# heyblackC/DFMIR

Hardware: AMD Instinct MI355X
Metric: train-step image-pairs/sec (fwd+bwd): 2D 256x256 bs=16 and 3D 160^3 bs=1 (higher is better)
Workload: dtype f32 (fp16x2-split MFMA, fp32 accumulate)

## Files before the change

dfmir_amd/_lib.py:

```python
import ctypes
import os
from ctypes import c_float, c_int, c_longlong, c_void_p, POINTER, Structure

_HERE = os.path.dirname(os.path.abspath(__file__))
LIB_PATH = os.environ.get("DFMIR_HIP_LIB") or os.path.join(_HERE, "libdfmir_hip.so")


class DfConvGeom(Structure):
    _fields_ = [(n, c_int) for n in (
        "N", "Cin", "Cout", "Di", "Hi", "Wi", "Do", "Ho", "Wo", "KD", "KH", "KW",
        "stride", "dil", "pd", "ph", "pw", "pad_mode", "act")] + [("slope", c_float)]


P = c_void_p
_GP = POINTER(DfConvGeom)
_SIGS = {
    "dfmir_abi_version": [],
    "dfmir_set_option": [ctypes.c_char_p, ctypes.c_char_p],
    "dfmir_get_option": [ctypes.c_char_p, ctypes.c_char_p, c_int],
    "dfmir_conv_fwd": [_GP, P, P, P, P, P],
    "dfmir_conv_wgrad": [_GP, P, P, P, P],
    "dfmir_bias_grad": [P, P, c_int, c_int, c_longlong, P],
    "dfmir_weight_pack": [P, P, c_int, c_int, c_int, c_int, P],
    "dfmir_weight_pack_floats": [c_int, c_int, c_int],
    "dfmir_weight_pack_batch": [P, c_int, P, c_int, P],
    "dfmir_conv3x3_res_ok": [_GP],
    "dfmir_conv3x3_fwd_scaled_res": [_GP, P, P, c_int, P, P, P, P, c_int, P, P],
    "dfmir_conv3x3_reflect_ring_ok": [_GP],
    "dfmir_conv3x3_reflect_ring_len": [_GP],
    "dfmir_conv3x3_reflect_ring": [_GP, P, P, P, c_int, P, P, P],
    "dfmir_conv_fwd_scaled": [_GP, P, P, c_int, P, P, P, P],
    "dfmir_conv_wgrad_scaled": [_GP, P, P, c_int, P, P, c_int, P, P, P],
    "dfmir_conv_wgrad_scaled_ch": [_GP, P, P, c_int, P, P, c_int, P, P, P, P],
    "dfmir_instnorm_bwd_pmax_ok": [c_longlong],
    "dfmir_instnorm_bwd_pmax": [P, P, P, P, P, c_int, c_longlong, c_int, P, P, c_int, P, P],
    "dfmir_patch_gather_bwd_gp": [P, P, P, c_int, c_int, c_longlong, c_int, c_int, P, P, P],
    "dfmir_patch_gather_bwd_any": [P, P, P, c_int, c_int, c_longlong, c_int, c_int, P, P, P],
    "dfmir_absmax": [P, c_longlong, P, P],
    "dfmir_conv3d_split_ok": [_GP],
    "dfmir_conv3d_split_ws_floats": [c_int, c_int],
    "dfmir_conv3d_split_fwd": [_GP, P, P, c_int, P, P, P, P, P, P],
    "dfmir_conv3d_split_fwd_sub": [_GP, P, P, c_int, P, P, P, P, P, c_int, P],
    "dfmir_conv3d_split_fwd_actgrad": [_GP, P, P, c_int, P, P, P, P, P, c_int, P, c_float, P],
    "dfmir_conv3d_up_ok": [c_int] * 6,
    "dfmir_conv3d_wsplit_batch": [P, c_int, P],
    "dfmir_conv3d_split_is_pair": [c_int],
    "dfmir_conv3d_march_ok": [_GP],
    "dfmir_conv3d_march_fwd": [_GP, P, P, c_int, P, P, P, P, P, c_float, P],
    "dfmir_conv3d_tiny_ok": [_GP],
    "dfmir_conv3d_tiny_fwd": [_GP, P, P, P, P, P, P, c_float, P],
    "dfmir_conv3d_s2c2_ok": [_GP],
    "dfmir_conv3d_s2c2_fwd": [_GP, P, P, P, P, P, P],
    "dfmir_conv3d_s2c2_wgrad": [_GP, P, P, P, P],
    "dfmir_conv3d_s2_ok": [_GP],
    "dfmir_conv3d_s2_fwd": [_GP, P, P, P, P, P, P],
    "dfmir_conv3d_s2_wgrad": [_GP, P, P, P, P, P],
    "dfmir_conv3d_s2_dgrad_ok": [_GP],
    "dfmir_conv3d_s2_dgrad": [_GP, P, P, P, P],
    "dfmir_conv3d_up_ws_floats": [c_int, c_int],
    "dfmir_conv3d_up_fwd": [P, P, c_int, P, c_int, P, P] + [c_int] * 6 + [P],
    "dfmir_conv3d_up_skip2_fwd": [P, P, c_int, P, P, c_int, c_int, P, P, P, P, P] + [c_int] * 7 + [c_float, P],
    "dfmir_conv3d_up_dgrad_ws_floats": [c_int, c_int],
    "dfmir_conv3d_up_dgrad": [P, P, c_int, P, c_int, P, P, P, P, c_float] + [c_int] * 6 + [P],
    "dfmir_conv3d_split_fwd_add": [_GP, P, P, c_int, P, c_int, c_int, P, P, P, P, P],
    "dfmir_conv3d_split_wgrad_ok": [_GP],
    "dfmir_conv3d_split_wgrad": [_GP, P, P, c_int, P, P, c_int, P, P],
    "dfmir_conv3d_split_wgrad_upcat": [_GP, P, P, c_int, P, c_int, P, P, c_int, P, P, P],
    "dfmir_conv3d_upwgrad_ok": [_GP, c_int],
    "dfmir_conv3d_wgrad_is_march": [_GP],
    "dfmir_conv3d_wgrad_is_march_at": [_GP, P, P],
    "dfmir_conv3d_upwgrad_ws_floats": [],
    "dfmir_conv3d_upwgrad": [_GP, P, P, c_int, P, c_int, P, P, c_int, P, P, P, P],
    "dfmir_conv3d_split_wgrad_db": [_GP, P, P, c_int, P, P, c_int, P, P, P],
    "dfmir_probe_merge": [P, P, P, P],
    "dfmir_act_bwd_amax": [P, P, P, c_longlong, c_int, c_float, P, P],
    "dfmir_weight_unpack": [P, P, c_int, c_int, c_int, P],
    "dfmir_weight_unpack_add_batch": [P, c_int, c_longlong, P],
    "dfmir_conv7x7_c1_fwd": [P, P, P, P, c_int, c_int, c_int, c_int, c_int, P],
    "dfmir_conv7x7_c1_wgrad": [P, P, P, P, c_int, c_int, c_int, c_int, c_int, P],
    "dfmir_tapstack_fwd": [P, P] + [c_int] * 7 + [P],
    "dfmir_tapstack_bwd": [P, P] + [c_int] * 7 + [P],
    "dfmir_tapsum_fwd": [P, P, P] + [c_int] * 10 + [c_float, P],
    "dfmir_tapsum_bwd": [P, P] + [c_int] * 9 + [P],
    "dfmir_instnorm_fwd": [P, P, P, P, P, c_int, c_longlong, c_float, c_int, P, P],
    "dfmir_instnorm_stats_ok": [c_longlong],
    "dfmir_instnorm_stats": [P, P, P, c_int, c_longlong, c_float, c_int, P, P],
    "dfmir_instnorm_bwd": [P, P, P, P, P, c_int, c_longlong, c_int, P, P],
    "dfmir_instnorm_bwd_cols_ok": [c_longlong, c_int],
    "dfmir_instnorm_bwd_cols": [P, P, P, P, P, c_int, c_longlong, c_int, P, P, c_int, P],
    "dfmir_in_relu_blurdown_ok": [c_int, c_int],
    "dfmir_in_relu_blurdown_fwd": [P, P, P, P, c_int, c_int, c_int, c_float, P, P],
    "dfmir_in_relu_blurdown_bwd": [P, P, P, P, P, c_int, c_int, c_int, P, P, P],
    "dfmir_act_bwd": [P, P, P, c_longlong, c_int, c_float, P],
    "dfmir_blur_down_fwd": [P, P, c_int, c_int, c_int, P],
    "dfmir_blur_down_bwd": [P, P, c_int, c_int, c_int, P],
    "dfmir_blur_up_fwd": [P, P, c_int, c_int, c_int, P],
    "dfmir_blur_up_bwd": [P, P, c_int, c_int, c_int, P],
    "dfmir_reflect_pad2d_fwd": [P, P, c_int, c_int, c_int, c_int, P],
    "dfmir_reflect_pad2d_bwd": [P, P, c_int, c_int, c_int, c_int, P],
    "dfmir_reflect_pad2d_bwd_add": [P, P, P, c_int, c_int, c_int, c_int, P],
    "dfmir_upcat_fwd": [P, P, P] + [c_int] * 7 + [P],
    "dfmir_upcat_bwd": [P, P, P] + [c_int] * 7 + [P],
    "dfmir_cat_channels_fwd": [P, P, P, c_longlong, c_longlong, c_longlong, P],
    "dfmir_cat_channels_bwd": [P, P, P, c_longlong, c_longlong, c_longlong, P],
    "dfmir_scale": [P, P, c_longlong, c_float, P],
    "dfmir_warp2d_fwd": [P, P, P] + [c_int] * 6 + [P],
    "dfmir_warp2d_bwd": [P, P, P, P, P] + [c_int] * 6 + [P],
    "dfmir_warp3d_fwd": [P, P, P] + [c_int] * 7 + [P],
    "dfmir_warp3d_bwd": [P, P, P, P, P] + [c_int] * 7 + [P],
    "dfmir_warp_bwd_own_ws_floats": [c_int] * 6,
    "dfmir_warp_bwd_own": [c_int, P, P, P, P, P] + [c_int] * 7 + [P, P],
    "dfmir_resize_fwd": [P, P] + [c_int] * 7 + [c_float, P],
    "dfmir_resize_bwd": [P, P] + [c_int] * 7 + [c_float, P],
    "dfmir_resize_bwd_ws_floats": [c_int] * 7,
    "dfmir_resize_bwd_sep": [P, P] + [c_int] * 7 + [c_float, P, P],
    "dfmir_patch_gather_fwd": [P, P, P, c_int, c_int, c_longlong, c_int, P],
    "dfmir_patch_gather_bwd": [P, P, P, c_int, c_int, c_longlong, c_int, P],
    "dfmir_patch_gather_bwd_amax": [P, P, P, c_int, c_int, c_longlong, c_int, P, P],
    "dfmir_patch_gather_fwd_g": [P, P, P, c_int, c_int, c_longlong, c_int, c_int, P],
    "dfmir_patch_gather_bwd_g": [P, P, P, c_int, c_int, c_longlong, c_int, c_int, P, P],
    "dfmir_l2norm_fwd": [P, P, P, c_int, c_longlong, c_float, P],
    "dfmir_l2norm_bwd": [P, P, P, P, c_int, c_longlong, c_float, P],
    "dfmir_patchnce_fwd": [P, P, P, P, c_longlong, c_int, c_int, c_float, P],
    "dfmir_patchnce_bwd": [P, P, P, P, c_longlong, c_int, c_int, c_float, P],
    "dfmir_masked_l1_fwd": [P, P, P, c_float, P, P, c_longlong, P],
    "dfmir_masked_l1_bwd": [P, P, P, c_float, P, P, P, P, c_longlong, P],
    "dfmir_flow_smooth_ws_floats": [],
    "dfmir_flow_smooth_fwd": [P, P, P] + [c_int] * 5 + [P],
    "dfmir_flow_smooth_bwd": [P, P, P] + [c_int] * 5 + [P],
    "dfmir_flow_smooth_fwd_p": [P, P, P] + [c_int] * 6 + [P],
    "dfmir_flow_smooth_bwd_p": [P, P, P] + [c_int] * 6 + [P],
    "dfmir_mul": [P, P, P, c_longlong, P],
    "dfmir_nmi_ws_floats": [c_longlong, c_int],
    "dfmir_nmi_fwd": [P, P, P, P, c_int, c_float, c_float, c_longlong, P, P, P],
    "dfmir_nmi_bwd": [P, P, P, P, c_int, c_float, c_float, c_longlong, P, P, P, P, P],
    "dfmir_ncc_fwd_m": [P, P, P, c_int, P, P, P, P] + [c_int] * 5 + [c_float, P],
    "dfmir_ncc_bwd_m": [P, P, P, c_int, P, P, P, P, P, P] + [c_int] * 5 + [c_float, P],
    "dfmir_ncc_fwd": [P, P, P, P, P, P] + [c_int] * 5 + [c_float, P],
    "dfmir_ncc_bwd": [P, P, P, P, P, P, P, P] + [c_int] * 5 + [c_float, P],
    "dfmir_patch_gather_fwd_multi": [P, c_int, P, P, c_int, c_int, c_longlong, c_int, P],
    "dfmir_nce_head_fwd": [P, c_int, P, P, P, P, P, P, P, P, P, P, c_int, c_int, c_longlong, c_int, c_float, P],
    "dfmir_patch_ids_draw": [P, P, c_int, c_int, c_int, P, P],
    "dfmir_segment_means_fwd": [P, P, c_int, c_int, c_longlong, c_float, P],
    "dfmir_segment_means_bwd": [P, P, c_int, c_int, c_longlong, c_float, P],
    "dfmir_scalar_combine_fwd": [P, c_int, P, c_int, P, P],
    "dfmir_scalar_combine_bwd": [P, c_int, P, c_int, P, P],
    "dfmir_det_head_floats": [],
    "dfmir_det_begin": [P, c_longlong, P, c_longlong, P, c_int, P, c_longlong, P, c_int, ctypes.c_double, P],
    "dfmir_det_end": [P, P, c_longlong, P, c_longlong, P],
    "dfmir_fill_zero": [P, c_longlong, P],
    "dfmir_sum_scaled": [P, P, c_longlong, c_float, P],
    "dfmir_fill_from_scalar": [P, P, c_longlong, c_float, P],
    "dfmir_adam_step": [P, P, P, P, c_longlong] + [c_float] * 7 + [P],
}

_lib = None


class DfmirHipError(RuntimeError):
    pass


def lib():
    global _lib
    if _lib is None:
        import torch
        if not os.path.exists(LIB_PATH):
            raise DfmirHipError(
                "libdfmir_hip.so not found at %s -- build it with `python -c 'import __graft_entry__ as g; "
                "g.build()'` or `make -C dfmir_amd/csrc` (there is no CPU fallback)" % LIB_PATH)
        h = ctypes.CDLL(LIB_PATH)
        for name, args in _SIGS.items():
            fn = getattr(h, name)
            fn.argtypes = args
            fn.restype = c_int
        h.dfmir_weight_pack_floats.restype = c_longlong
        h.dfmir_conv3d_split_ws_floats.restype = c_longlong
        h.dfmir_conv3d_up_ws_floats.restype = c_longlong
        h.dfmir_conv3d_up_dgrad_ws_floats.restype = c_longlong
        h.dfmir_conv3d_upwgrad_ws_floats.restype = c_longlong
        h.dfmir_flow_smooth_ws_floats.restype = c_longlong
        h.dfmir_nmi_ws_floats.restype = c_longlong
        h.dfmir_warp_bwd_own_ws_floats.restype = c_longlong
        h.dfmir_resize_bwd_ws_floats.restype = c_longlong
        h.dfmir_last_error.argtypes = []
        h.dfmir_last_error.restype = ctypes.c_char_p
        _lib = h
    return _lib


def check(rc):
    if rc != 0:
        msg = lib().dfmir_last_error()
        raise DfmirHipError(msg.decode() if msg else "dfmir_hip error %d" % rc)


def set_option(name, value=None):
    check(lib().dfmir_set_option(name.encode(), None if value is None else str(value).encode()))


def get_option(name):
    buf = ctypes.create_string_buffer(256)
    n = lib().dfmir_get_option(name.encode(), buf, 256)
    return None if n < 0 else buf.value.decode()


def exported_symbols():
    return sorted(list(_SIGS.keys()) + ["dfmir_last_error"])
```

dfmir_amd/csrc/taps.hip:

```cpp
#include "common.h"

__device__ __forceinline__ int pre_images(int i, int n, int pad, int pad_mode, int* rp) {
  int cnt = 0;
  rp[cnt++] = i;
  if (pad_mode == 1) {
    if (i >= 1 && i <= pad) rp[cnt++] = -i;
    if (i <= n - 2 && i >= n - 1 - pad) rp[cnt++] = 2 * (n - 1) - i;
  }
  return cnt;
}
__device__ __forceinline__ bool map_coord(int c, int n, int pad_mode, int& out) {
  if (pad_mode == 1) {
    if (c < 0) c = -c;
    if (c >= n) c = 2 * (n - 1) - c;
    out = c < 0 ? 0 : (c >= n ? n - 1 : c);
    return true;
  }
  out = c;
  return (unsigned)c < (unsigned)n;
}

__global__ void tapstack_fwd_k(const float* __restrict__ x, float* __restrict__ s, int N, int C, int H, int W,
                               int K, int pad, int pad_mode) {
  const int T = K * K;
// ... 173 lines not shown
  const int co = mb * 32 + l31;
  float a[25];
#pragma unroll
  for (int s2 = 0; s2 < 25; ++s2) {
    const int t = 2 * s2 + lhi;
    a[s2] = (t < S7_T && co < Cout) ? w[co * S7_T + t] : 0.f;
  }
  __syncthreads();
  st_f32x16 acc[S7_RW];
#pragma unroll
  for (int j = 0; j < S7_RW; ++j)
#pragma unroll
    for (int r = 0; r < 16; ++r) acc[j][r] = 0.f;
#pragma unroll
  for (int s2 = 0; s2 < 25; ++s2) {
    const int t = 2 * s2 + lhi < S7_T ? 2 * s2 + lhi : S7_T - 1;
    const int off = (t / S7_K) * S7_PW + (t % S7_K) + l31;
#pragma unroll
    for (int j = 0; j < S7_RW; ++j)
      acc[j] = __builtin_amdgcn_mfma_f32_32x32x2f32(patch[(rg * S7_RW + j) * S7_PW + off], a[s2], acc[j], 0, 0, 0);
  }
  float* yn = y + (long long)n * Cout * H * W;
  const float bz = (bias && co < Cout) ? bias[co] : 0.f;
  const bool vec = (W & 3) == 0 && ((reinterpret_cast<unsigned long long>(y) & 15) == 0);
  if (co < Cout) {
#pragma unroll
    for (int j = 0; j < S7_RW; ++j) {
      const int oy = ty0 + rg * S7_RW + j;
      if (oy >= H) continue;
      float* row = yn + ((long long)co * H + oy) * W;
#pragma unroll
      for (int q = 0; q < 4; ++q) {
        const int ox = tx0 + 8 * q + 4 * lhi;
        if (ox >= W) continue;
        const float v0 = acc[j][4 * q] + bz, v1 = acc[j][4 * q + 1] + bz, v2 = acc[j][4 * q + 2] + bz, v3 = acc[j][4 * q + 3] + bz;
        if (vec) *reinterpret_cast<float4*>(row + ox) = make_float4(v0, v1, v2, v3);
        else {
          row[ox] = v0;
          if (ox + 1 < W) row[ox + 1] = v1;
          if (ox + 2 < W) row[ox + 2] = v2;
          if (ox + 3 < W) row[ox + 3] = v3;
        }
      }
    }
  }
}

constexpr int S7W_TH = 8, S7W_PH = S7W_TH + 6;
__global__ __launch_bounds__(256) void conv7x7_c1_wgrad_k(const float* __restrict__ x, const float* __restrict__ dy,
                                                          float* __restrict__ dw, float* __restrict__ db,
                                                          int N, int H, int W, int Cout, int pad_mode,
                                                          int tiles_x, int tiles_y, const float* __restrict__ fx) {
  __shared__ float patch[S7W_PH * S7_PW];
  __shared__ float dyt[64 * (S7W_TH * S7_TW + 1)];
  constexpr int DS = S7W_TH * S7_TW + 1;
  const int tid = threadIdx.x, lane = tid & 63, wid = tid >> 6;
  const int l31 = lane & 31, lhi = lane >> 5;
  const int mb = wid & 1, tb = wid >> 1;
  const int t = tb * 32 + l31;
  const int tc = t < S7_T ? t : S7_T - 1;
  const int toff = (tc / S7_K) * S7_PW + (tc % S7_K);
  st_f32x16 acc;
#pragma unroll
  for (int r = 0; r < 16; ++r) acc[r] = 0.f;
  const long long HW = (long long)H * W;
  const int ntile = N * tiles_y * tiles_x;
  for (int tl = blockIdx.x; tl < ntile; tl += gridDim.x) {
    const int n = tl / (tiles_y * tiles_x), q = tl - n * tiles_y * tiles_x;
    const int ty0 = (q / tiles_x) * S7W_TH, tx0 = (q % tiles_x) * S7_TW;
    const float* xn = x + (long long)n * HW;
    const float* dyn = dy + (long long)n * Cout * HW;
    __syncthreads();
    for (int i = tid; i < S7W_PH * S7_PW; i += 256) {
      const int r = i / S7_PW, c = i - r * S7_PW;
      const int o = s7_src(ty0 + r - 3, tx0 + c - 3, H, W, pad_mode);
      patch[i] = o >= 0 ? xn[o] : 0.f;
    }
    {
      float4 ld[16];
#pragma unroll
      for (int q4 = 0; q4 < 16; ++q4) {
        const int i4 = tid + 256 * q4, c = i4 >> 6, r4 = i4 & 63;
        const int oy = ty0 + (r4 >> 3), ox = tx0 + ((r4 & 7) << 2);
        const float* src = dyn + ((long long)c * H + oy) * W + ox;
        if (c < Cout && oy < H && ox + 3 < W && (W & 3) == 0) ld[q4] = *reinterpret_cast<const float4*>(src);
        else {
          ld[q4].x = (c < Cout && oy < H && ox < W) ? src[0] : 0.f;
          ld[q4].y = (c < Cout && oy < H && ox + 1 < W) ? src[1] : 0.f;
          ld[q4].z = (c < Cout && oy < H && ox + 2 < W) ? src[2] : 0.f;
          ld[q4].w = (c < Cout && oy < H && ox + 3 < W) ? src[3] : 0.f;
        }
      }
#pragma unroll
      for (int q4 = 0; q4 < 16; ++q4) {
        const int i4 = tid + 256 * q4, c = i4 >> 6, px = (i4 & 63) << 2;
        float* d = dyt + c * DS + px;
        d[0] = ld[q4].x; d[1] = ld[q4].y; d[2] = ld[q4].z; d[3] = ld[q4].w;
      }
    }
    __syncthreads();
    constexpr int G = 16, NG = S7W_TH * S7_TW / (2 * G);
    float av[2][G], bv[2][G];
    const float* arow = dyt + (mb * 32 + l31) * DS + lhi;
#define S7W_LOAD(set_, g_)                                                                       \
    _Pragma("unroll") for (int e = 0; e < G; ++e) {                                              \
      const int px = 2 * ((g_) * G + e) + lhi;                                                   \
      av[set_][e] = arow[2 * ((g_) * G + e)];                                                    \
      bv[set_][e] = t == S7_T ? 1.f : patch[(px >> 5) * S7_PW + (px & 31) + toff];               \
    }
    S7W_LOAD(0, 0)
#pragma unroll
    for (int g = 0; g < NG; ++g) {
      if (g + 1 < NG) S7W_LOAD((g + 1) & 1, g + 1)
#pragma unroll
      for (int e = 0; e < G; ++e)
        acc = __builtin_amdgcn_mfma_f32_32x32x2f32(av[g & 1][e], bv[g & 1][e], acc, 0, 0, 0);
    }
#undef S7W_LOAD
  }
  if (t <= S7_T) {
#pragma unroll
    for (int r = 0; r < 16; ++r) {
      const int c = mb * 32 + 4 * lhi + (r & 3) + 8 * (r >> 2);
      if (c < Cout) {
        if (t < S7_T) df_acc(dw, c * S7_T + t, acc[r], fx);
        else if (db) df_acc(db, c, acc[r], fx);
      }
    }
  }
}

extern "C" int dfmir_conv7x7_c1_fwd(const float* x, const float* w, const float* bias, float* y, int N, int H, int W,
                                    int Cout, int pad_mode, void* stream) {
  DF_ARG_CHECK(x && w && y && N > 0 && N <= 65535 && H >= 4 && W >= 4 && Cout > 0 && Cout <= 64);
  DF_ARG_CHECK(pad_mode == 0 || pad_mode == 1);
  const int tx = (W + S7_TW - 1) / S7_TW, ty = (H + S7_TH - 1) / S7_TH;
  conv7x7_c1_fwd_k<<<dim3((unsigned)(tx * ty), (unsigned)N), 256, 0, (hipStream_t)stream>>>(x, w, bias, y, H, W, Cout,
                                                                                           pad_mode, tx);
  DF_LAUNCH_CHECK();
  return 0;
}
extern "C" int dfmir_conv7x7_c1_wgrad(const float* x, const float* dy, float* dw, float* db, int N, int H, int W,
                                      int Cout, int pad_mode, void* stream) {
  DF_ARG_CHECK(x && dy && dw && N > 0 && H >= 4 && W >= 4 && Cout > 0 && Cout <= 64);
  DF_ARG_CHECK(pad_mode == 0 || pad_mode == 1);
  const int tx = (W + S7_TW - 1) / S7_TW, ty = (H + S7W_TH - 1) / S7W_TH;
  const long long ntile = (long long)N * tx * ty;
  DF_ARG_CHECK(ntile < (1LL << 31));
  const unsigned grid = (unsigned)(ntile < 512 ? ntile : 512);
  conv7x7_c1_wgrad_k<<<grid, 256, 0, (hipStream_t)stream>>>(x, dy, dw, db, N, H, W, Cout, pad_mode, tx, ty, df_det_fx());
  DF_LAUNCH_CHECK();
  return 0;
}
```

dfmir_amd/ops.py:

```python
import ctypes
import os

import torch
from torch.autograd import Function
from torch.autograd.function import once_differentiable

from ._lib import DfConvGeom, DfmirHipError, check, lib

_VP = ctypes.c_void_p


def _p(t):
    return None if t is None else _VP(t.data_ptr())


def _st():
    return _VP(torch.cuda.current_stream().cuda_stream)


def _need(*ts):
    for t in ts:
        if t is None:
            continue
        if not t.is_cuda:
# ... 725 lines not shown
                else:
                    check(lib().dfmir_reflect_pad2d_bwd(_p(dxp), _p(dx5), x5.shape[0] * Cin, in_sp[1], in_sp[2],
                                                        p3[1], _st()))
            else:
                padp = tuple(K[i] - 1 - p3[i] for i in range(3))
                used = Cin - ctx.dead_tail if (ctx.dead_tail and stride == 1 and not _NO_DEAD_TAIL) else None
                ia = ctx.in_act if (stride == 1 and nd == 3) else None
                dx5 = conv_raw(dy5, wd, None, Cin, K, 1, padp, stride, 0, 0, 0.0, in_sp, dy_amax, cout_used=used,
                               act_src=x5 if ia else None, act_slope=ia[1] if ia else 0.0)
                if ia and _LAST_ACTGRAD[0]:
                    dx5._df_premasked = (dx5._version, dx5.data_ptr())
            dx = dx5 if nd == 3 else dx5.squeeze(2)
        if dskip is not None:
            dx = dskip if dx is None else dx + dskip
        defer = (_DEFER["on"] and owner is not None and getattr(owner, "weight", None) is not None
                 and owner.weight.grad is not None and owner.weight.grad.is_contiguous())
        db_buf = None
        if ctx.has_bias and ctx.needs_input_grad[2]:
            bg = getattr(owner, "bias", None).grad if defer and getattr(owner, "bias", None) is not None else None
            if bg is not None and bg.is_contiguous():
                db_buf = bg
            else:
                db = db_buf = zeros(Cout, dy5.device)
        if ctx.needs_input_grad[1]:
            ptag = getattr(dy, "_df_pmax", None) if not act else None
            dy_pmax = ptag[0] if (ptag is not None and ptag[1] == dy._version and ptag[2] == dy.data_ptr()
                                  and dy.is_contiguous() and not _NO_CH_SCALE) else None
            parts = getattr(ctx, "x_parts", None)
            if defer:
                T = K[0] * K[1] * K[2]
                conv_wgrad_raw(x5, dy5, K, stride, p3, pad_mode,
                               out=_deferred_buffer(owner, T, Cin, Cout, tuple(weight.shape), dy5.device),
                               x_amax=ctx.x_amax, dy_amax=dy_amax, db=db_buf, dy_pmax=dy_pmax, parts=parts)
            else:
                dwt = conv_wgrad_raw(x5, dy5, K, stride, p3, pad_mode, x_amax=ctx.x_amax, dy_amax=dy_amax, db=db_buf,
                                     dy_pmax=dy_pmax, parts=parts)
                dw = weight_unpack(dwt, tuple(weight.shape))
        elif db_buf is not None:
            bias_grad(dy5, db_buf)
        return dx, dw, db


_LAST_CONV_AMAX = [None]


def conv(x, weight, bias=None, owner=None, stride=1, pad=0, pad_mode=0, act=0, slope=0.0, skip=False, sole=False):
    _LAST_CONV_AMAX[0] = None
    out = ConvFn.apply(x, weight, bias, owner, stride, pad, pad_mode, act, slope, skip)
    if _LAST_CONV_AMAX[0] is not None and not skip:
        tag_amax(out, _LAST_CONV_AMAX[0])
        _LAST_CONV_AMAX[0] = None
    if sole and act == 1 and not skip and x.dim() == 5:
        out._df_act_sole = (act, float(slope), out._version, out.data_ptr())
    return out


class TapStackFn(Function):

    @staticmethod
    def forward(ctx, x, K, pad, pad_mode):
        _need(x)
        x = _c(x)
        N, C, H, W = x.shape
        s = torch.empty((N, C * K * K, H, W), device=x.device, dtype=torch.float32)
        check(lib().dfmir_tapstack_fwd(_p(x), _p(s), N, C, H, W, K, pad, pad_mode, _st()))
        ctx.meta = (N, C, H, W, K, pad, pad_mode)
        return s

    @staticmethod
    @once_differentiable
    def backward(ctx, ds):
        N, C, H, W, K, pad, pad_mode = ctx.meta
        ds = _c(ds)
        dx = torch.empty((N, C, H, W), device=ds.device, dtype=torch.float32)
        check(lib().dfmir_tapstack_bwd(_p(ds), _p(dx), N, C, H, W, K, pad, pad_mode, _st()))
        return dx, None, None, None


class TapSumFn(Function):

    @staticmethod
    def forward(ctx, z, bias, C, K, pad, pad_mode, act, slope):
        _need(z, bias)
        z = _c(z)
        N, CT, H, W = z.shape
        y = torch.empty((N, C, H, W), device=z.device, dtype=torch.float32)
        check(lib().dfmir_tapsum_fwd(_p(z), _p(bias), _p(y), N, C, H, W, H, W, K, pad, pad_mode, act, float(slope), _st()))
        ctx.meta = (N, C, H, W, K, pad, pad_mode, act, float(slope))
        ctx.save_for_backward(y if act else None)
        ctx.has_bias = bias is not None
        return y

    @staticmethod
    @once_differentiable
    def backward(ctx, dy):
        N, C, H, W, K, pad, pad_mode, act, slope = ctx.meta
        (y,) = ctx.saved_tensors
        dy = _c(dy)
        if act:
            dpre = torch.empty_like(dy)
            check(lib().dfmir_act_bwd(_p(dy), _p(y), _p(dpre), dy.numel(), act, slope, _st()))
            dy = dpre
        dz = db = None
        if ctx.needs_input_grad[0]:
            dz = torch.empty((N, C * K * K, H, W), device=dy.device, dtype=torch.float32)
            check(lib().dfmir_tapsum_bwd(_p(dy), _p(dz), N, C, H, W, H, W, K, pad, pad_mode, _st()))
        if ctx.has_bias and ctx.needs_input_grad[1]:
            db = zeros(C, dy.device)
            bias_grad(dy.view(N, C, H * W), db)
        return dz, db, None, None, None, None, None, None


class Stem7Fn(Function):

    @staticmethod
    def forward(ctx, x, weight, bias, pad_mode):
        _need(x, weight, bias)
        x = _c(x)
        N, _, H, W = x.shape
        Cout = weight.shape[0]
        y = torch.empty((N, Cout, H, W), device=x.device, dtype=torch.float32)
        check(lib().dfmir_conv7x7_c1_fwd(_p(x), _p(_c(weight)), _p(bias), _p(y), N, H, W, Cout, pad_mode, _st()))
        ctx.save_for_backward(x, weight)
        ctx.pad_mode = pad_mode
        ctx.has_bias = bias is not None
        return y

    @staticmethod
    @once_differentiable
    def backward(ctx, dy):
        x, weight = ctx.saved_tensors
        dy = _c(dy)
        N, _, H, W = x.shape
        Cout = weight.shape[0]
        dx = dw = db = None
        if ctx.needs_input_grad[1] or (ctx.has_bias and ctx.needs_input_grad[2]):
            dwb = zeros(Cout * 49 + Cout, dy.device)
            dbp = dwb[Cout * 49:] if ctx.has_bias else None
            if _DET["on"]:
                det = _DetAcc(Cout * 49, Cout if ctx.has_bias else 0, N * H * W, x, None, dy, None)
                try:
                    check(lib().dfmir_conv7x7_c1_wgrad(_p(x), _p(dy), _p(det.dw), None, N, H, W, Cout, ctx.pad_mode, _st()))
                    if ctx.has_bias:
                        check(lib().dfmir_bias_grad(_p(dy), _p(det.db), N, Cout, H * W, _st()))
                except BaseException:
                    det.abort()
                    raise
                det.end(dwb, dbp)
            else:
                check(lib().dfmir_conv7x7_c1_wgrad(_p(x), _p(dy), _p(dwb), _p(dbp), N, H, W, Cout, ctx.pad_mode, _st()))
            dw = dwb[:Cout * 49].view(Cout, 1, 7, 7)
            db = dbp if (ctx.has_bias and ctx.needs_input_grad[2]) else None
        if ctx.needs_input_grad[0]:
            wd = weight_pack(weight.detach().view(Cout, 49, 1), 1)
            ds = conv_raw(dy.unsqueeze(2), wd, None, 49, (1, 1, 1), 1, (0, 0, 0), 1, 0, 0, 0.0, (1, H, W))
            dx = torch.empty_like(x)
            check(lib().dfmir_tapstack_bwd(_p(ds), _p(dx), N, 1, H, W, 7, 3, ctx.pad_mode, _st()))
        return dx, dw, db, None


_NO_STEM7 = _env_on("DFMIR_NO_STEM7")


def conv_taps(x, weight, bias, pad, pad_mode, act=0, slope=0.0):
    Cout, Cin, K = weight.shape[0], weight.shape[1], weight.shape[2]
    T = K * K
    if Cin == 1 and K == 7 and pad == 3 and Cout <= 64 and act == 0 and x.dim() == 4 and not _NO_STEM7:
        return Stem7Fn.apply(x, weight, bias, pad_mode)
    if Cin == 1:
        s = TapStackFn.apply(x, K, pad, pad_mode)
        return conv(s, weight.view(Cout, T, 1, 1), bias, None, 1, 0, 0, act, slope)
    wz = weight.view(Cout, Cin, T).permute(0, 2, 1).reshape(Cout * T, Cin, 1, 1)
    z = conv(x, wz, None, None, 1, 0, 0, 0, 0.0)
    return TapSumFn.apply(z, bias, Cout, K, pad, pad_mode, act, slope)


class InstNormFn(Function):
    @staticmethod
    def forward(ctx, x, res, relu, eps):
        _need(x, res)
        x = _c(x)
        planes = x.shape[0] * x.shape[1]
        S = x.numel() // planes
        y = torch.empty_like(x)
        mean = torch.empty(planes, device=x.device, dtype=torch.float32)
        rstd = torch.empty_like(mean)
        r = _c(res) if res is not None else None
        slot = amax_slot(x.device, PROBE_SLOTS)
        check(lib().dfmir_instnorm_fwd(_p(x), _p(r), _p(y), _p(mean), _p(rstd), planes, S, float(eps),
                                       int(relu), _p(slot), _st()))
        _LAST_AMAX[0] = slot
        ctx.save_for_backward(x, mean, rstd)
        ctx.relu = int(relu)
        ctx.has_res = res is not None
        return y

    @staticmethod
    @once_differentiable
    def backward(ctx, dy):
        x, mean, rstd = ctx.saved_tensors
        dy = _c(dy)
        planes = x.shape[0] * x.shape[1]
        S = x.numel() // planes
        dx = None
        if ctx.needs_input_grad[0]:
            dx = torch.empty_like(x)
            slot = amax_slot(x.device, PROBE_SLOTS)
            W = x.shape[-1]
            want_cols = x.dim() == 4 and W <= 94 and S // W <= 94 and lib().dfmir_instnorm_bwd_cols_ok(S, W)
            cols = torch.empty(planes * 2 * (S // W), device=x.device, dtype=torch.float32) if want_cols else None
            if x.dim() == 4 and lib().dfmir_instnorm_bwd_pmax_ok(S):
                pmax = torch.empty(planes, device=x.device, dtype=torch.float32)
                check(lib().dfmir_instnorm_bwd_pmax(_p(dy), _p(x), _p(mean), _p(rstd), _p(dx), planes, S, ctx.relu,
                                                    _p(slot), _p(cols), W if want_cols else 0, _p(pmax), _st()))
                dx._df_pmax = (pmax, dx._version, dx.data_ptr())
            elif want_cols:
                check(lib().dfmir_instnorm_bwd_cols(_p(dy), _p(x), _p(mean), _p(rstd), _p(dx), planes, S, ctx.relu,
                                                    _p(slot), _p(cols), W, _st()))
            else:
                check(lib().dfmir_instnorm_bwd(_p(dy), _p(x), _p(mean), _p(rstd), _p(dx), planes, S, ctx.relu,
                                               _p(slot), _st()))
            if want_cols:
                dx._df_cols = (cols, dx._version, dx.data_ptr())
            tag_amax(dx, slot)
        dres = dy if (ctx.has_res and ctx.needs_input_grad[1]) else None
        return dx, dres, None, None


_LAST_AMAX = [None]


def instance_norm(x, res=None, relu=False, eps=1e-5):
    y = InstNormFn.apply(x, res, relu, eps)
    return tag_amax(y, _LAST_AMAX[0])


_NO_IN_BLUR = _env_on("DFMIR_NO_IN_BLUR")


class InstNormReluBlurDownFn(Function):

    @staticmethod
    def forward(ctx, x, eps):
        _need(x)
        x = _c(x)
        N, C, H, W = x.shape
        planes = N * C
        z = torch.empty((N, C, H // 2, W // 2), device=x.device, dtype=torch.float32)
        mean = torch.empty(planes, device=x.device, dtype=torch.float32)
        rstd = torch.empty_like(mean)
        slot = amax_slot(x.device, PROBE_SLOTS)
        check(lib().dfmir_in_relu_blurdown_fwd(_p(x), _p(z), _p(mean), _p(rstd), planes, H, W, float(eps), _p(slot), _st()))
        _LAST_AMAX[0] = slot
        ctx.save_for_backward(x, mean, rstd)
        return z

    @staticmethod
    @once_differentiable
    def backward(ctx, dz):
        x, mean, rstd = ctx.saved_tensors
        dz = _c(dz)
        N, C, H, W = x.shape
        dx = torch.empty_like(x)
        slot = amax_slot(x.device, PROBE_SLOTS)
        pmax = torch.empty(N * C, device=x.device, dtype=torch.float32)
        check(lib().dfmir_in_relu_blurdown_bwd(_p(dz), _p(x), _p(mean), _p(rstd), _p(dx), N * C, H, W, _p(slot), _p(pmax),
                                               _st()))
        dx._df_pmax = (pmax, dx._version, dx.data_ptr())
        tag_amax(dx, slot)
        return dx, None


def in_relu_blurdown_ok(x):
    return (not _NO_IN_BLUR and x.dim() == 4 and x.is_cuda and x.dtype == torch.float32
            and bool(lib().dfmir_in_relu_blurdown_ok(int(x.shape[2]), int(x.shape[3]))))


def instance_norm_relu_blur_down(x, eps=1e-5):
    z = InstNormReluBlurDownFn.apply(x, eps)
    return tag_amax(z, _LAST_AMAX[0])


def _plane_op(fwd_name, bwd_name, out_hw):
    class _Fn(Function):
        @staticmethod
        def forward(ctx, x, *extra):
            _need(x)
            x = _c(x)
            N, C, H, W = x.shape
            Ho, Wo = out_hw(H, W, *extra)
            y = torch.empty((N, C, Ho, Wo), device=x.device, dtype=torch.float32)
            check(getattr(lib(), fwd_name)(_p(x), _p(y), N * C, H, W, *extra, _st()))
            ctx.shape = (N, C, H, W)
            ctx.extra = extra
            return y

        @staticmethod
        @once_differentiable
        def backward(ctx, dy):
            N, C, H, W = ctx.shape
            dy = _c(dy)
            dx = torch.empty((N, C, H, W), device=dy.device, dtype=torch.float32)
            check(getattr(lib(), bwd_name)(_p(dy), _p(dx), N * C, H, W, *ctx.extra, _st()))
            return (dx,) + (None,) * len(ctx.extra)

    _Fn.__name__ = fwd_name
    return _Fn


BlurDownFn = _plane_op("dfmir_blur_down_fwd", "dfmir_blur_down_bwd",
                       lambda H, W: ((H - 1) // 2 + 1, (W - 1) // 2 + 1))
BlurUpFn = _plane_op("dfmir_blur_up_fwd", "dfmir_blur_up_bwd", lambda H, W: (2 * H, 2 * W))
ReflectPadFn = _plane_op("dfmir_reflect_pad2d_fwd", "dfmir_reflect_pad2d_bwd",
                         lambda H, W, p: (H + 2 * p, W + 2 * p))
# ... 1214 lines not shown
```

include/dfmir_hip.h:

```cpp
#ifndef DFMIR_HIP_H
#define DFMIR_HIP_H

#ifdef __cplusplus
extern "C" {
#endif

#define DFMIR_ABI_VERSION 14

int dfmir_abi_version(void);
const char* dfmir_last_error(void);

int dfmir_set_option(const char* name, const char* value);
int dfmir_get_option(const char* name, char* buf, int buf_len);

typedef struct DfConvGeom {
  int N, Cin, Cout;
  int Di, Hi, Wi;
  int Do, Ho, Wo;
  int KD, KH, KW;
  int stride, dil;
  int pd, ph, pw;
  int pad_mode;
  int act;
  float slope;
} DfConvGeom;

int dfmir_conv_fwd(const DfConvGeom* g, const float* x, const float* w_tcc, const float* bias,
                   float* y, void* stream);
int dfmir_conv_fwd_scaled(const DfConvGeom* g, const float* x, const float* x_amax, int x_amax_n,
                          const float* w_tcc, const float* bias, float* y, void* stream);
#define DFMIR_PROBE_SLOTS 64
int dfmir_absmax(const float* x, long long n, float* out, void* stream);
int dfmir_conv3d_split_ok(const DfConvGeom* g);
long long dfmir_conv3d_split_ws_floats(int Cin, int Cout);
int dfmir_conv3d_split_fwd(const DfConvGeom* g, const float* x, const float* x_amax, int x_amax_n, const float* w_tcc,
                           float* ws, const float* bias, float* y, float* y_amax, void* stream);
int dfmir_conv3d_split_fwd_sub(const DfConvGeom* g, const float* x, const float* x_amax, int x_amax_n, const float* w_tcc,
                               float* ws, const float* bias, float* y, float* y_amax, int cout_used, void* stream);
int dfmir_conv3d_split_fwd_actgrad(const DfConvGeom* g, const float* x, const float* x_amax, int x_amax_n,
                                   const float* w_tcc, float* ws, const float* bias, float* y, float* y_amax,
                                   int cout_used, const float* act_src, float act_slope, void* stream);
int dfmir_conv3d_up_ok(int N, int Ca, int Cout, int D, int H, int W);
int dfmir_conv3d_wsplit_batch(const void* jobs_dev, int njobs, void* stream);
int dfmir_conv3d_split_is_pair(int cout_used);
int dfmir_conv3d_march_ok(const DfConvGeom* g);
int dfmir_conv3d_march_fwd(const DfConvGeom* g, const float* x, const float* x_amax, int x_amax_n, const float* w_tcc,
                           const float* bias, float* y, float* y_amax, const float* act_src, float act_slope,
                           void* stream);
int dfmir_conv3d_tiny_ok(const DfConvGeom* g);
int dfmir_conv3d_tiny_fwd(const DfConvGeom* g, const float* x, const float* w_tcc, const float* bias, float* y,
                          float* y_amax, const float* act_src, float act_slope, void* stream);
int dfmir_conv3d_s2c2_ok(const DfConvGeom* g);
int dfmir_conv3d_s2c2_fwd(const DfConvGeom* g, const float* x, const float* w_tcc, const float* bias, float* y, float* y_amax,
                          void* stream);
int dfmir_conv3d_s2c2_wgrad(const DfConvGeom* g, const float* x, const float* dy, float* dw_tcc, void* stream);
int dfmir_conv3d_s2_ok(const DfConvGeom* g);
int dfmir_conv3d_s2_fwd(const DfConvGeom* g, const float* x, const float* w_tcc, const float* bias, float* y, float* y_amax,
                        void* stream);
int dfmir_conv3d_s2_wgrad(const DfConvGeom* g, const float* x, const float* dy, float* dw_tcc, float* db, void* stream);
int dfmir_conv3d_s2_dgrad_ok(const DfConvGeom* g);
int dfmir_conv3d_s2_dgrad(const DfConvGeom* g, const float* dy, const float* w_tcc, float* dx, void* stream);
long long dfmir_conv3d_up_ws_floats(int Ca, int Cout);
int dfmir_conv3d_up_fwd(const float* a, const float* a_amax, int a_amax_n, const float* w_tcc, int Ktot, float* ws,
                        float* y, int N, int Ca, int Cout, int D, int H, int W, void* stream);
int dfmir_conv3d_up_skip2_fwd(const float* a, const float* a_amax, int a_amax_n, const float* b, const float* b_amax,
                              int b_amax_n, int Cb, const float* w_tcc, float* ws, const float* bias, float* y,
                              float* y_amax, int N, int Ca, int Cout, int D, int H, int W, int act, float slope,
                              void* stream);
long long dfmir_conv3d_up_dgrad_ws_floats(int Ca, int Cout);
int dfmir_conv3d_up_dgrad(const float* dy, const float* dy_amax, int dy_amax_n, const float* w_tcc, int Ktot, float* ws,
                          float* da, float* da_amax, const float* act_src, float act_slope, int N, int Ca, int Cout, int D,
                          int H, int W, void* stream);
int dfmir_conv3d_split_fwd_add(const DfConvGeom* g, const float* b, const float* b_amax, int b_amax_n, const float* w_tcc,
                               int Ktot, int koff, float* ws, const float* bias, float* y, float* y_amax, void* stream);
int dfmir_conv3d_split_wgrad_ok(const DfConvGeom* g);
int dfmir_conv3d_split_wgrad(const DfConvGeom* g, const float* x, const float* x_amax, int x_amax_n, const float* dy,
                             const float* dy_amax, int dy_amax_n, float* dw_tcc, void* stream);
int dfmir_conv3d_split_wgrad_upcat(const DfConvGeom* g, const float* a, const float* b, int Ca, const float* x_amax,
                                   int x_amax_n, const float* dy, const float* dy_amax, int dy_amax_n, float* dw_tcc,
                                   float* db, void* stream);
int dfmir_conv3d_upwgrad_ok(const DfConvGeom* g, int Ca);
long long dfmir_conv3d_upwgrad_ws_floats(void);
int dfmir_conv3d_upwgrad(const DfConvGeom* g, const float* a, const float* b, int Ca, const float* x_amax, int x_amax_n,
                         const float* dy, const float* dy_amax, int dy_amax_n, float* dw_tcc, float* db, float* ws,
                         void* stream);
int dfmir_conv3d_split_wgrad_db(const DfConvGeom* g, const float* x, const float* x_amax, int x_amax_n, const float* dy,
                                const float* dy_amax, int dy_amax_n, float* dw_tcc, float* db, void* stream);
int dfmir_conv3d_wgrad_is_march(const DfConvGeom* g);
int dfmir_conv3d_wgrad_is_march_at(const DfConvGeom* g, const float* x, const float* dy);
int dfmir_probe_merge(const float* a, const float* b, float* out, void* stream);
int dfmir_conv_wgrad(const DfConvGeom* g, const float* x, const float* dy, float* dw_tcc,
                     void* stream);
int dfmir_conv_wgrad_scaled(const DfConvGeom* g, const float* x, const float* x_amax, int x_amax_n,
                            const float* dy, const float* dy_amax, int dy_amax_n, float* dw_tcc, float* db,
                            void* stream);
int dfmir_conv_wgrad_scaled_ch(const DfConvGeom* g, const float* x, const float* x_amax, int x_amax_n, const float* dy,
                               const float* dy_amax, int dy_amax_n, const float* dy_pmax, float* dw_tcc, float* db,
                               void* stream);
int dfmir_bias_grad(const float* dy, float* db, int N, int C, long long S, void* stream);
long long dfmir_weight_pack_floats(int Cout, int Cin, int T);
int dfmir_weight_pack(const float* w, float* w_tcc, int Cout, int Cin, int T, int mode, void* stream);
int dfmir_weight_unpack(const float* g_tcc, float* g, int Cout, int Cin, int T, void* stream);
int dfmir_conv3x3_res_ok(const DfConvGeom* g);
int dfmir_conv3x3_fwd_scaled_res(const DfConvGeom* g, const float* x, const float* x_amax, int x_amax_n,
                                 const float* w_tcc, const float* bias, const float* res, const float* ring,
                                 int ring_len, float* y, void* stream);

int dfmir_conv3x3_reflect_ring_ok(const DfConvGeom* g);
int dfmir_conv3x3_reflect_ring_len(const DfConvGeom* g);
int dfmir_conv3x3_reflect_ring(const DfConvGeom* g, const float* dy, const float* dy_cols, const float* dy_amax,
                               int dy_amax_n, const float* wd_packed, float* ring, void* stream);

typedef struct DfPackJob {
  const float* w;
  float* packed;
  int Cout, Cin, T, mode;
} DfPackJob;
int dfmir_weight_pack_batch(const DfPackJob* jobs, int njobs, void* table_dev, int upload, void* stream);

typedef struct DfUnpackJob {
  float* src;
  float* dst;
  int Cout, Cin, T, reserved;
} DfUnpackJob;
int dfmir_weight_unpack_add_batch(const DfUnpackJob* jobs, int njobs, long long max_total, void* stream);

int dfmir_conv7x7_c1_fwd(const float* x, const float* w, const float* bias, float* y, int N, int H, int W, int Cout,
                         int pad_mode, void* stream);
int dfmir_conv7x7_c1_wgrad(const float* x, const float* dy, float* dw, float* db, int N, int H, int W, int Cout,
                           int pad_mode, void* stream);

int dfmir_tapstack_fwd(const float* x, float* s, int N, int C, int H, int W, int K, int pad,
                       int pad_mode, void* stream);
int dfmir_tapstack_bwd(const float* ds, float* dx, int N, int C, int H, int W, int K, int pad,
                       int pad_mode, void* stream);
int dfmir_tapsum_fwd(const float* z, const float* bias, float* y, int N, int C, int Hz, int Wz, int Ho,
                     int Wo, int K, int opad, int pad_mode, int act, float slope, void* stream);
int dfmir_tapsum_bwd(const float* dy, float* dz, int N, int C, int Hz, int Wz, int Ho, int Wo, int K,
                     int opad, int pad_mode, void* stream);

int dfmir_instnorm_stats_ok(long long S);
int dfmir_instnorm_stats(const float* x, float* mean, float* rstd, int planes, long long S, float eps, int relu,
                         float* y_amax, void* stream);
int dfmir_instnorm_fwd(const float* x, const float* res, float* y, float* mean, float* rstd,
                       int planes, long long S, float eps, int relu, float* y_amax, void* stream);
int dfmir_instnorm_bwd(const float* dy, const float* x, const float* mean, const float* rstd,
                       float* dx, int planes, long long S, int relu, float* dx_amax, void* stream);
int dfmir_instnorm_bwd_cols_ok(long long S, int W);
int dfmir_instnorm_bwd_cols(const float* dy, const float* x, const float* mean, const float* rstd, float* dx, int planes,
                            long long S, int relu, float* dx_amax, float* dx_cols, int W, void* stream);
int dfmir_instnorm_bwd_pmax_ok(long long S);
int dfmir_instnorm_bwd_pmax(const float* dy, const float* x, const float* mean, const float* rstd, float* dx, int planes,
                            long long S, int relu, float* dx_amax, float* dx_cols, int W, float* dx_pmax, void* stream);

int dfmir_in_relu_blurdown_ok(int H, int W);
int dfmir_in_relu_blurdown_fwd(const float* x, float* z, float* mean, float* rstd, int planes, int H, int W, float eps,
                               float* z_amax, void* stream);
int dfmir_in_relu_blurdown_bwd(const float* dz, const float* x, const float* mean, const float* rstd, float* dx,
                               int planes, int H, int W, float* dx_amax, float* dx_pmax, void* stream);

int dfmir_act_bwd(const float* dy, const float* y, float* dx, long long n, int act, float slope,
                  void* stream);
int dfmir_act_bwd_amax(const float* dy, const float* y, float* dx, long long n, int act, float slope,
                       float* dx_amax, void* stream);

int dfmir_blur_down_fwd(const float* x, float* y, int planes, int H, int W, void* stream);
int dfmir_blur_down_bwd(const float* dy, float* dx, int planes, int H, int W, void* stream);
int dfmir_blur_up_fwd(const float* x, float* y, int planes, int H, int W, void* stream);
int dfmir_blur_up_bwd(const float* dy, float* dx, int planes, int H, int W, void* stream);
int dfmir_reflect_pad2d_fwd(const float* x, float* y, int planes, int H, int W, int p, void* stream);
int dfmir_reflect_pad2d_bwd(const float* dy, float* dx, int planes, int H, int W, int p, void* stream);
int dfmir_reflect_pad2d_bwd_add(const float* dy, const float* add, float* dx, int planes, int H, int W, int p,
                                void* stream);

int dfmir_upcat_fwd(const float* a, const float* b, float* y, int N, int Ca, int Cb, int Da, int Ha,
                    int Wa, int sd, void* stream);
int dfmir_upcat_bwd(const float* dy, float* da, float* db, int N, int Ca, int Cb, int Da, int Ha,
                    int Wa, int sd, void* stream);

int dfmir_cat_channels_fwd(const float* a, const float* b, float* y, long long N, long long SA,
                           long long SB, void* stream);
int dfmir_cat_channels_bwd(const float* dy, float* da, float* db, long long N, long long SA,
                           long long SB, void* stream);
int dfmir_scale(const float* x, float* y, long long n, float mult, void* stream);

int dfmir_warp2d_fwd(const float* src, const float* flow, float* out, int B, int C, int H, int W,
                     int mode, int add_identity, void* stream);
int dfmir_warp2d_bwd(const float* dout, const float* src, const float* flow, float* dsrc,
                     float* dflow, int B, int C, int H, int W, int add_identity, int flow_into_src,
                     void* stream);
int dfmir_warp3d_fwd(const float* src, const float* flow, float* out, int B, int C, int D, int H,
                     int W, int mode, int add_identity, void* stream);
int dfmir_warp3d_bwd(const float* dout, const float* src, const float* flow, float* dsrc,
                     float* dflow, int B, int C, int D, int H, int W, int add_identity,
                     int flow_into_src, void* stream);
long long dfmir_warp_bwd_own_ws_floats(int nd, int B, int C, int D, int H, int W);
int dfmir_warp_bwd_own(int nd, const float* dout, const float* src, const float* flow, float* dsrc, float* dflow, int B,
                       int C, int D, int H, int W, int add_identity, int flow_into_src, float* ws, void* stream);

int dfmir_resize_fwd(const float* x, float* y, int planes, int Di, int Hi, int Wi, int Do, int Ho,
                     int Wo, float mult, void* stream);
int dfmir_resize_bwd(const float* dy, float* dx, int planes, int Di, int Hi, int Wi, int Do, int Ho,
                     int Wo, float mult, void* stream);
long long dfmir_resize_bwd_ws_floats(int planes, int Di, int Hi, int Wi, int Do, int Ho, int Wo);
int dfmir_resize_bwd_sep(const float* dy, float* dx, int planes, int Di, int Hi, int Wi, int Do, int Ho, int Wo,
                         float mult, float* ws, void* stream);

int dfmir_patch_gather_fwd(const float* feat, const long long* ids, float* out, int B, int C,
                           long long S, int P, void* stream);
int dfmir_patch_gather_bwd(const float* dout, const long long* ids, float* dfeat, int B, int C,
                           long long S, int P, void* stream);
int dfmir_patch_gather_bwd_amax(const float* dout, const long long* ids, float* dfeat, int B, int C, long long S,
                                int P, float* dfeat_amax, void* stream);
int dfmir_patch_gather_fwd_g(const float* feat, const long long* ids, float* out, int B, int C, long long S, int P,
                             int G, void* stream);
int dfmir_patch_gather_bwd_g(const float* dout, const long long* ids, float* dfeat, int B, int C, long long S, int P,
                             int G, float* dfeat_amax, void* stream);
int dfmir_patch_gather_bwd_gp(const float* dout, const long long* ids, float* dfeat, int B, int C, long long S, int P,
                              int G, float* dfeat_amax, float* dfeat_pmax, void* stream);
int dfmir_patch_gather_bwd_any(const float* dout, const long long* ids, float* dfeat, int B, int C, long long S, int P,
                               int G, float* dfeat_amax, float* dfeat_pmax, void* stream);
int dfmir_patch_gather_fwd_multi(const float* const* srcs, int G, const long long* ids, float* out, int Bper, int C,
                                 long long S, int P, void* stream);
int dfmir_nce_head_fwd(const float* const* srcs, int G, const long long* ids, const float* w1, const float* b1,
                       const float* w2, const float* b2, float* out, float* nrm, float* xs, float* hs, float* ypre,
                       int Bper, int C, long long S, int P, float eps, void* stream);
int dfmir_patch_ids_draw(unsigned long long* state, const long long* sizes, int n_layers, int n_sets, int P,
                         long long* out, void* stream);
int dfmir_l2norm_fwd(const float* x, float* y, float* norm, int C, long long rows, float eps, void* stream);
int dfmir_l2norm_bwd(const float* dy, const float* x, const float* norm, float* dx, int C,
                     long long rows, float eps, void* stream);
int dfmir_patchnce_fwd(const float* q, const float* k, float* loss, float* probs, long long rows,
                       int C, int G, float T, void* stream);
int dfmir_patchnce_bwd(const float* dloss, const float* probs, const float* k, float* dq,
                       long long rows, int C, int G, float T, void* stream);

int dfmir_masked_l1_fwd(const float* a, const float* b, const unsigned char* mask, float thr,
                        float* ws, float* out, long long n, void* stream);
int dfmir_masked_l1_bwd(const float* a, const float* b, const unsigned char* mask, float thr,
                        const float* ws, const float* gout, float* da, float* db, long long n,
                        void* stream);
long long dfmir_flow_smooth_ws_floats(void);
int dfmir_flow_smooth_fwd(const float* flow, float* ws, float* out, int B, int C, int D, int H,
                          int W, void* stream);
int dfmir_flow_smooth_bwd(const float* flow, const float* gout, float* dflow, int B, int C, int D,
                          int H, int W, void* stream);
int dfmir_flow_smooth_fwd_p(const float* flow, float* ws, float* out, int B, int C, int D, int H,
                            int W, int penalty, void* stream);
int dfmir_flow_smooth_bwd_p(const float* flow, const float* gout, float* dflow, int B, int C, int D,
                            int H, int W, int penalty, void* stream);
long long dfmir_nmi_ws_floats(long long n, int nb);
int dfmir_nmi_fwd(const float* y_true, const float* y_pred, const float* mask, const float* centers, int nb,
                  float preterm, float max_clip, long long n, float* ws, float* out, void* stream);
int dfmir_nmi_bwd(const float* y_true, const float* y_pred, const float* mask, const float* centers, int nb,
                  float preterm, float max_clip, long long n, const float* ws, const float* gout, float* d_true,
                  float* d_pred, void* stream);
int dfmir_mul(const float* a, const float* b, float* out, long long n, void* stream);
int dfmir_ncc_fwd(const float* I, const float* J, float* tmp, float* tmp2, float* ws, float* out,
                  int B, int D, int H, int W, int win, float eps, void* stream);
int dfmir_ncc_bwd(const float* I, const float* J, const float* sums, float* tmp, float* tmp2,
                  const float* ws, const float* gout, float* dI, int B, int D, int H, int W,
                  int win, float eps, void* stream);
int dfmir_ncc_fwd_m(const float* I, const float* J, const float* mask, int mode, float* tmp, float* tmp2,
                    float* ws, float* out, int B, int D, int H, int W, int win, float eps, void* stream);
int dfmir_ncc_bwd_m(const float* I, const float* J, const float* mask, int mode, const float* sums,
                    float* tmp, float* tmp2, const float* ws, const float* gout, float* dI, int B, int D,
                    int H, int W, int win, float eps, void* stream);
int dfmir_segment_means_fwd(const float* rows, float* out, int L, int T, long long seg, float scale, void* stream);
int dfmir_segment_means_bwd(const float* gout, float* drows, int L, int T, long long seg, float scale, void* stream);
int dfmir_scalar_combine_fwd(const float* const* in, int n_in, const float* M, int n_out, float* out, void* stream);
int dfmir_scalar_combine_bwd(const float* gout, int n_in, const float* M, int n_out, float* din, void* stream);
int dfmir_fill_zero(float* p, long long n, void* stream);
int dfmir_sum_scaled(const float* x, float* out, long long n, float scale, void* stream);
int dfmir_fill_from_scalar(const float* gout, float* dx, long long n, float scale, void* stream);

int dfmir_det_head_floats(void);
int dfmir_det_begin(float* scratch, long long slots, const float* x, long long nx, const float* x_amax, int x_amax_n,
                    const float* dy, long long ndy, const float* dy_amax, int dy_amax_n, double count, void* stream);
int dfmir_det_end(const float* scratch, float* dw_out, long long n_dw, float* db_out, long long n_db, void* stream);

int dfmir_adam_step(float* p, const float* g, float* m, float* v, long long n, float lr, float beta1,
                    float beta2, float eps, float bc1, float bc2, float grad_scale, void* stream);

// ... 5 lines not shown
```

Before: 213.3.

## Fuse 7x7 single-channel stem dgrad into one MFMA kernel with LDS tap-sum

Replaces the stem conv's input-gradient path. It used to pack the weights, run a generic 1x1 conv to produce a 49-tap stack in global memory, then call tapstack_bwd. Now a dedicated kernel computes the per-tap channel contractions with split-fp16 MFMA into shared memory and sums the taps, including reflect-pad folding, before writing dx directly. This removes the intermediate 49xHxW tensor round trip and two extra launches. It costs a bespoke kernel with per-row dynamic fp16 scaling, which may differ slightly in precision from the old path. An environment flag keeps the old path available.

```diff
diff --git a/dfmir_amd/_lib.py b/dfmir_amd/_lib.py
--- a/dfmir_amd/_lib.py
+++ b/dfmir_amd/_lib.py
@@ -78,6 +78,7 @@
     "dfmir_weight_unpack_add_batch": [P, c_int, c_longlong, P],
     "dfmir_conv7x7_c1_fwd": [P, P, P, P, c_int, c_int, c_int, c_int, c_int, P],
     "dfmir_conv7x7_c1_wgrad": [P, P, P, P, c_int, c_int, c_int, c_int, c_int, P],
+    "dfmir_conv7x7_c1_dgrad": [P, P, P, c_int, c_int, c_int, c_int, c_int, P],
     "dfmir_tapstack_fwd": [P, P] + [c_int] * 7 + [P],
     "dfmir_tapstack_bwd": [P, P] + [c_int] * 7 + [P],
     "dfmir_tapsum_fwd": [P, P, P] + [c_int] * 10 + [c_float, P],
diff --git a/dfmir_amd/csrc/taps.hip b/dfmir_amd/csrc/taps.hip
--- a/dfmir_amd/csrc/taps.hip
+++ b/dfmir_amd/csrc/taps.hip
@@ -349,3 +349,147 @@
   DF_LAUNCH_CHECK();
   return 0;
 }
+
+typedef _Float16 d7_f16x8 __attribute__((ext_vector_type(8)));
+constexpr int D7_TH = 6, D7_TW = 26, D7_HH = D7_TH + 6, D7_HW = 32, D7_PL = D7_HH * D7_HW, D7_THREADS = 256;
+
+__device__ __forceinline__ float d7_wave_max(float v) {
+#pragma unroll
+  for (int o = 32; o > 0; o >>= 1) v = fmaxf(v, __shfl_xor(v, o));
+  return v;
+}
+__device__ __forceinline__ float d7_scale(float amax) {
+  if (!(amax > 0.f) || !(amax < 3.0e38f)) return 1.f;
+  int e;
+  frexpf(amax, &e);
+  e = e < -100 ? -100 : e;
+  return ldexpf(1.f, 15 - e);
+}
+__device__ __forceinline__ void d7_split(const float* v, float s, d7_f16x8& h, d7_f16x8& l) {
+#pragma unroll
+  for (int j = 0; j < 8; ++j) {
+    const float a = v[j] * s;
+    const _Float16 hj = (_Float16)a;
+    h[j] = hj;
+    l[j] = (_Float16)(a - (float)hj);
+  }
+}
+
+__global__ __launch_bounds__(D7_THREADS) void conv7x7_c1_dgrad_k(const float* __restrict__ dy,
+                                                               const float* __restrict__ w, float* __restrict__ dx,
+                                                               int N, int C, int H, int W, int pad_mode, int tiles_x,
+                                                               int tiles_y) {
+  __shared__ float z[S7_T * D7_PL];
+  const int tid = threadIdx.x, lane = tid & 63, wid = tid >> 6;
+  const int l31 = lane & 31, lhi = lane >> 5;
+  d7_f16x8 wh[2][4], wl[2][4];
+  float sw;
+  {
+    float wv[2][4][8], m = 0.f;
+#pragma unroll
+    for (int tb = 0; tb < 2; ++tb)
+#pragma unroll
+      for (int ks = 0; ks < 4; ++ks)
+#pragma unroll
+        for (int j = 0; j < 8; ++j) {
+          const int t = 32 * tb + l31, c = 16 * ks + 8 * lhi + j;
+          wv[tb][ks][j] = (t < S7_T && c < C) ? w[c * S7_T + t] : 0.f;
+          m = fmaxf(m, fabsf(wv[tb][ks][j]));
+        }
+    sw = d7_scale(d7_wave_max(m));
+#pragma unroll
+    for (int tb = 0; tb < 2; ++tb)
+#pragma unroll
+      for (int ks = 0; ks < 4; ++ks) d7_split(wv[tb][ks], sw, wh[tb][ks], wl[tb][ks]);
+  }
+  const long long HW = (long long)H * W;
+  const int ntile = N * tiles_y * tiles_x;
+  for (int tl = blockIdx.x; tl < ntile; tl += gridDim.x) {
+    const int n = tl / (tiles_y * tiles_x), q = tl - n * tiles_y * tiles_x;
+    const int ty0 = (q / tiles_x) * D7_TH, tx0 = (q % tiles_x) * D7_TW;
+    const float* dyn = dy + (long long)n * C * HW;
+    for (int hr = wid; hr < D7_HH; hr += D7_THREADS / 64) {
+      const int gy = ty0 - 3 + hr, gx = tx0 - 3 + l31;
+      const int off = ((unsigned)gy < (unsigned)H && (unsigned)gx < (unsigned)W) ? gy * W + gx : -1;
+      float xv[4][8], m = 0.f;
+#pragma unroll
+      for (int ks = 0; ks < 4; ++ks)
+#pragma unroll
+        for (int j = 0; j < 8; ++j) {
+          const int c = 16 * ks + 8 * lhi + j;
+          xv[ks][j] = (off >= 0 && c < C) ? dyn[(long long)c * HW + off] : 0.f;
+          m = fmaxf(m, fabsf(xv[ks][j]));
+        }
+      const float sx = d7_scale(d7_wave_max(m));
+      d7_f16x8 xh[4], xl[4];
+#pragma unroll
+      for (int ks = 0; ks < 4; ++ks) d7_split(xv[ks], sx, xh[ks], xl[ks]);
+      const float inv = (1.f / sw) * (1.f / sx);
+#pragma unroll
+      for (int tb = 0; tb < 2; ++tb) {
+        st_f32x16 acc;
+#pragma unroll
+        for (int r = 0; r < 16; ++r) acc[r] = 0.f;
+#pragma unroll
+        for (int ks = 0; ks < 4; ++ks) {
+          acc = __builtin_amdgcn_mfma_f32_32x32x16_f16(wh[tb][ks], xh[ks], acc, 0, 0, 0);
+          acc = __builtin_amdgcn_mfma_f32_32x32x16_f16(wh[tb][ks], xl[ks], acc, 0, 0, 0);
+          acc = __builtin_amdgcn_mfma_f32_32x32x16_f16(wl[tb][ks], xh[ks], acc, 0, 0, 0);
+        }
+#pragma unroll
+        for (int r = 0; r < 16; ++r) {
+          const int t = 32 * tb + 8 * (r >> 2) + 4 * lhi + (r & 3);
+          if (t < S7_T) z[t * D7_PL + hr * D7_HW + l31] = acc[r] * inv;
+        }
+      }
+    }
+    __syncthreads();
+    if (tid < D7_TH * D7_TW) {
+      const int r = tid / D7_TW, c = tid - r * D7_TW;
+      const int py = ty0 + r, px = tx0 + c;
+      if (py < H && px < W) {
+        float s = 0.f;
+        for (int kh = 0; kh < S7_K; ++kh)
+#pragma unroll
+          for (int kw = 0; kw < S7_K; ++kw) s += z[(kh * S7_K + kw) * D7_PL + (r + 6 - kh) * D7_HW + c + 6 - kw];
+        if (pad_mode == 1 && (py <= 3 || py >= H - 4 || px <= 3 || px >= W - 4)) {
+          for (int a = 0; a < 3; ++a) {
+            const int ry = a == 0 ? py : (a == 1 ? (py >= 1 && py <= 3 ? -py : INT_MIN)
+                                                 : (py <= H - 2 && py >= H - 4 ? 2 * (H - 1) - py : INT_MIN));
+            if (ry == INT_MIN) continue;
+            for (int b = 0; b < 3; ++b) {
+              if (a == 0 && b == 0) continue;
+              const int rx = b == 0 ? px : (b == 1 ? (px >= 1 && px <= 3 ? -px : INT_MIN)
+                                                   : (px <= W - 2 && px >= W - 4 ? 2 * (W - 1) - px : INT_MIN));
+              if (rx == INT_MIN) continue;
+              for (int kh = 0; kh < S7_K; ++kh) {
+                const int oy = ry - kh + 3, hy = oy - ty0 + 3;
+                if ((unsigned)oy >= (unsigned)H || (unsigned)hy >= (unsigned)D7_HH) continue;
+                for (int kw = 0; kw < S7_K; ++kw) {
+                  const int ox = rx - kw + 3, hx = ox - tx0 + 3;
+                  if ((unsigned)ox < (unsigned)W && (unsigned)hx < (unsigned)D7_HW)
+                    s += z[(kh * S7_K + kw) * D7_PL + hy * D7_HW + hx];
+                }
+              }
+            }
+          }
+        }
+        dx[(long long)n * HW + (long long)py * W + px] = s;
+      }
+    }
+    __syncthreads();
+  }
+}
+
+extern "C" int dfmir_conv7x7_c1_dgrad(const float* dy, const float* w, float* dx, int N, int H, int W, int Cout,
+                                      int pad_mode, void* stream) {
+  DF_ARG_CHECK(dy && w && dx && N > 0 && H >= 4 && W >= 4 && Cout > 0 && Cout <= 64);
+  DF_ARG_CHECK(pad_mode == 0 || pad_mode == 1);
+  const int tx = (W + D7_TW - 1) / D7_TW, ty = (H + D7_TH - 1) / D7_TH;
+  const long long ntile = (long long)N * tx * ty;
+  DF_ARG_CHECK(ntile < (1LL << 31));
+  const unsigned grid = (unsigned)(ntile < 512 ? ntile : 512);
+  conv7x7_c1_dgrad_k<<<grid, D7_THREADS, 0, (hipStream_t)stream>>>(dy, w, dx, N, Cout, H, W, pad_mode, tx, ty);
+  DF_LAUNCH_CHECK();
+  return 0;
+}
diff --git a/dfmir_amd/ops.py b/dfmir_amd/ops.py
--- a/dfmir_amd/ops.py
+++ b/dfmir_amd/ops.py
@@ -901,14 +901,18 @@
             dw = dwb[:Cout * 49].view(Cout, 1, 7, 7)
             db = dbp if (ctx.has_bias and ctx.needs_input_grad[2]) else None
         if ctx.needs_input_grad[0]:
-            wd = weight_pack(weight.detach().view(Cout, 49, 1), 1)
-            ds = conv_raw(dy.unsqueeze(2), wd, None, 49, (1, 1, 1), 1, (0, 0, 0), 1, 0, 0, 0.0, (1, H, W))
             dx = torch.empty_like(x)
-            check(lib().dfmir_tapstack_bwd(_p(ds), _p(dx), N, 1, H, W, 7, 3, ctx.pad_mode, _st()))
+            if _NO_STEM7_DGRAD:
+                wd = weight_pack(weight.detach().view(Cout, 49, 1), 1)
+                ds = conv_raw(dy.unsqueeze(2), wd, None, 49, (1, 1, 1), 1, (0, 0, 0), 1, 0, 0, 0.0, (1, H, W))
+                check(lib().dfmir_tapstack_bwd(_p(ds), _p(dx), N, 1, H, W, 7, 3, ctx.pad_mode, _st()))
+            else:
+                check(lib().dfmir_conv7x7_c1_dgrad(_p(dy), _p(_c(weight)), _p(dx), N, H, W, Cout, ctx.pad_mode, _st()))
         return dx, dw, db, None
 
 
 _NO_STEM7 = _env_on("DFMIR_NO_STEM7")
+_NO_STEM7_DGRAD = _env_on("DFMIR_NO_STEM7_DGRAD")
 
 
 def conv_taps(x, weight, bias, pad, pad_mode, act=0, slope=0.0):
diff --git a/include/dfmir_hip.h b/include/dfmir_hip.h
--- a/include/dfmir_hip.h
+++ b/include/dfmir_hip.h
@@ -129,6 +129,8 @@
                          int pad_mode, void* stream);
 int dfmir_conv7x7_c1_wgrad(const float* x, const float* dy, float* dw, float* db, int N, int H, int W, int Cout,
                            int pad_mode, void* stream);
+int dfmir_conv7x7_c1_dgrad(const float* dy, const float* w, float* dx, int N, int H, int W, int Cout, int pad_mode,
+                           void* stream);
 
 int dfmir_tapstack_fwd(const float* x, float* s, int N, int C, int H, int W, int K, int pad,
                        int pad_mode, void* stream);
```

Result: no change. 214.0 (median of 6 runs) (+0.3%).
